# nhchiu/Shadow-Removal-ISTD

Measured on AMD Instinct MI355X. Metric: ST-CGAN train images/s at 256×256 bs=32, 1/2/4/8 MI355X; G2 max-abs vs CPU, higher is better.
Workload: dtype bf16; 1 GPU; full ST-CGAN train step (G1,G2,D1,D2 fwd/bwd + MSE-cGAN/L1 + Adam), 256x256; global_batch=32, per_gpu_batch=32, image_size=256, ngf=64, parallelism=dp1, step_launch=eager

## Files before the change

include/stcgan_hip.h:

```cpp
#ifndef STCGAN_HIP_H
#define STCGAN_HIP_H

#include <stdint.h>

#ifdef __cplusplus
extern "C" {
#endif

enum { STC_F32 = 0, STC_BF16 = 1 };

typedef struct {
  void* p;
  int32_t H, W;
  int64_t bs;
  int64_t rs;
  int32_t ps;
  int32_t co;
  int32_t cs;
  int32_t pad_;
} stc_view;

enum { STC_CONV_S2 = 0, STC_CONV_S1 = 1, STC_CONVT_S2 = 2, STC_CONV_S1_DGRAD = 3 };

int stc_conv_fwd(int dtype, int kind, int B,
// ... 41 lines not shown
                    float* running_var, int64_t* num_batches_tracked, float momentum, float eps, stc_view apply_x,
                    stc_view y1, float slope1, stc_view y2, float slope2, void* workspace, int64_t workspace_bytes,
                    void* stream);

int stc_conv_bwd_act_ok(int dtype, int kind, int B, stc_view dy, int Cin, int Cout, stc_view out, stc_view x,
                        stc_view g_other);
int stc_conv_bwd_act(int dtype, int kind, int B, stc_view dy, int Cin, const void* w_packed, int Cout,
                     stc_view out, stc_view x, float slope_self, stc_view g_other, float slope_other, void* stream);

int stc_conv_fwd_act_ok(int dtype, int kind, int B, stc_view x, int Cin, int Cout, stc_view y1, stc_view y2);
int stc_conv_fwd_act(int dtype, int kind, int B, stc_view x, int Cin, const void* w_packed, int Cout,
                     stc_view y1, float slope1, stc_view y2, float slope2, const float* bias,
                     void* workspace, int64_t workspace_bytes, void* stream);

int stc_set_splitk_inlaunch(int on);

int stc_conv_wgrad(int dtype, int B, int stride,
                   stc_view D, int R,
                   const float* d_scale, const float* d_shift, int d_act, float d_slope,
                   stc_view G, int Cg, int Cg_out,
                   const float* g_scale, const float* g_shift, int g_act, float g_slope,
                   float* dW, void* workspace, int64_t workspace_bytes, void* stream);
int64_t stc_conv_wgrad_workspace(int dtype, int B, int Hd, int Wd, int R, int Cg);
int stc_conv_wgrad_ex(int dtype, int B, int stride,
                      stc_view D, int R,
                      const float* d_scale, const float* d_shift, int d_act, float d_slope,
                      stc_view G, int Cg, int Cg_out,
                      const float* g_scale, const float* g_shift, int g_act, float g_slope,
                      float* dW, const int32_t* force_plan, void* workspace, int64_t workspace_bytes, void* stream);
int stc_conv_wgrad_query(int dtype, int B, int Hd, int Wd, int R, int Cg, const int32_t* force_plan,
// ... 197 lines not shown
```

shadow-removal-istd_amd/csrc/bn.hip:

```cpp
#include <type_traits>

#include "common.hpp"
#include "philox.hpp"

namespace stc {

constexpr int STAT_PIX = 64;

__host__ __device__ inline int stat_chunks(long long P) {
  long long c = (P + STAT_PIX - 1) / STAT_PIX;
  if (c > 1024) c = 1024;
  if (c < 1) c = 1;
  return (int)c;
}

template <typename T> struct VW;
template <> struct VW<float> {
  static constexpr int N = 4;
  __device__ __forceinline__ static void load(const float* p, float* f) {
    const float4 v = *reinterpret_cast<const float4*>(p);
    f[0] = v.x; f[1] = v.y; f[2] = v.z; f[3] = v.w;
  }
  __device__ __forceinline__ static void store(float* p, const float* f) {
    *reinterpret_cast<float4*>(p) = make_float4(f[0], f[1], f[2], f[3]);
// ... 186 lines not shown
    }
    sm = mu;
  }
  const double N = n, mu = sm;
  const double M2 = block_sum256(m2, sh);
  if (threadIdx.x == 0)
    bn_finalize_store(c, N, mu, M2, pre, rmean, rvar, nbt, momentum, eps, mean_o, rstd_o, scale, shift);
}

__device__ __forceinline__ double wave_sum(double v) {
#pragma unroll
  for (int o = 32; o > 0; o >>= 1) v += __shfl_xor(v, o, 64);
  return v;
}

__global__ void __launch_bounds__(256) bn_finalize_wave_kernel(const float* part, int nchunks, int C,
                                                               const float* gamma, const float* beta,
                                                               float* rmean, float* rvar, long long* nbt,
                                                               float momentum, float eps,
                                                               float* mean_o, float* rstd_o, float* scale, float* shift) {
  const int lane = threadIdx.x & 63;
  const int c = blockIdx.x * 4 + (threadIdx.x >> 6);
  if (c >= C) return;
  auto load4 = [&](int k0, float4* pp) {
#pragma unroll
    for (int u = 0; u < 4; ++u) {
      const int k = k0 + u * 64;
      pp[u] = k < nchunks ? *reinterpret_cast<const float4*>(part + ((long long)k * C + c) * 4)
                          : make_float4(0.f, 0.f, 0.f, 0.f);
    }
  };
  const BnPre pre = bn_pre(c, gamma, beta, rmean, rvar);
  auto sum1 = [&](const float4* pp, double& n, double& sm) {
#pragma unroll
    for (int u = 0; u < 4; ++u) {
      if (pp[u].x <= 0.f) continue;
      n += pp[u].x;
      sm += (double)pp[u].x * pp[u].w + (double)pp[u].y;
    }
  };
  auto sum2 = [&](const float4* pp, double mu, double& m2) {
#pragma unroll
    for (int u = 0; u < 4; ++u) {
      if (pp[u].x <= 0.f) continue;
      const double nb = pp[u].x, s1 = pp[u].y, r = s1 / nb;
      double q = (double)pp[u].z - s1 * r;
      if (q < 0) q = 0;
// ... 25 lines not shown
  } else {
    for (int k0 = lane; k0 < nchunks; k0 += 256) {
      float4 pp[4];
      load4(k0, pp);
      sum1(pp, n, sm);
    }
    n = wave_sum(n);
    sm = wave_sum(sm);
    mu = n > 0 ? sm / n : 0.0;
    for (int k0 = lane; k0 < nchunks; k0 += 256) {
      float4 pp[4];
      load4(k0, pp);
      sum2(pp, mu, m2);
    }
  }
  const double M2 = wave_sum(m2);
  if (lane == 0) bn_finalize_store(c, n, mu, M2, pre, rmean, rvar, nbt, momentum, eps, mean_o, rstd_o, scale, shift);
}

__global__ void bn_eval_table_kernel(int C, const float* gamma, const float* beta, const float* rmean,
                                     const float* rvar, float eps, float* scale, float* shift) {
  const int c = blockIdx.x * blockDim.x + threadIdx.x;
  if (c >= C) return;
  const float rs = 1.f / sqrtf(rvar[c] + eps);
  const float sc = gamma[c] * rs;
  scale[c] = sc;
  shift[c] = beta[c] - rmean[c] * sc;
}

struct GradIn {
  View g1, g2;
// ... 95 lines not shown
    }
#pragma unroll
    for (int u = 0; u < 4; ++u) {
      a += pp[u].x;
      b += pp[u].y;
    }
  }
  const double ta = block_sum256(a, sh);
  const double tb = block_sum256(b, sh);
  if (threadIdx.x == 0) {
    dbeta[c] = (float)ta;
    dgamma[c] = (float)tb;
  }
}

__global__ void __launch_bounds__(256) bn_bwd_finalize_wave_kernel(const float* part, int nchunks, int C, float* dgamma,
                                                                   float* dbeta) {
  const int lane = threadIdx.x & 63;
  const int c = blockIdx.x * 4 + (threadIdx.x >> 6);
  if (c >= C) return;
  double a = 0, b = 0;
  for (int k0 = lane; k0 < nchunks; k0 += 256) {
    float2 pp[4];
#pragma unroll
    for (int u = 0; u < 4; ++u) {
      const int k = k0 + u * 64;
      pp[u] = k < nchunks ? *reinterpret_cast<const float2*>(part + ((long long)k * C + c) * 2) : make_float2(0.f, 0.f);
    }
#pragma unroll
    for (int u = 0; u < 4; ++u) {
      a += pp[u].x;
      b += pp[u].y;
    }
  }
  a = wave_sum(a);
  b = wave_sum(b);
  if (lane == 0) {
    dbeta[c] = (float)a;
    dgamma[c] = (float)b;
  }
}

template <typename T, bool DENSE>
__global__ void __launch_bounds__(256) bn_bwd_apply_kernel(View x, PixDiv pd, long long P, int C, const float* scale,
                                                           const float* shift, const float* mean, const float* rstd,
                                                           const float* gamma, GradIn gi, const float* dgamma,
                                                           const float* dbeta, View dx) {
  constexpr int N = VW<T>::N;
  const int CG = C / N;
  const long long total = P * CG;
  const long long stride = (long long)gridDim.x * blockDim.x;
  const float invP = 1.f / (float)P;
  int cg_have = -1;
  float sc[N], sh[N], k0[N], k1[N], k2[N];
  auto table = [&](int cg) {
    if (cg == cg_have) return;
    cg_have = cg;
    const int c = N * cg;
    if (scale) { ldc<N>(scale + c, sc); ldc<N>(shift + c, sh); }
    else {
#pragma unroll
      for (int e = 0; e < N; ++e) { sc[e] = 1.f; sh[e] = 0.f; }
    }
    if (mean) {
      float mu[N], rs[N], gm[N], dg[N], db[N];
      ldc<N>(mean + c, mu); ldc<N>(rstd + c, rs); ldc<N>(gamma + c, gm); ldc<N>(dgamma + c, dg); ldc<N>(dbeta + c, db);
#pragma unroll
      for (int e = 0; e < N; ++e) {
        k1[e] = gm[e] * rs[e];
        k2[e] = k1[e] * rs[e] * dg[e] * invP;
        k0[e] = k1[e] * (db[e] * invP - mu[e] * rs[e] * dg[e] * invP);
      }
    } else {
#pragma unroll
      for (int e = 0; e < N; ++e) { k1[e] = 1.f; k2[e] = 0.f; k0[e] = 0.f; }
    }
  };
  struct Off {
    long long x, g1, g2, dx;
    int c;
  };
  auto offs = [&](long long idx) {
    Off o;
    const int cg = (int)(idx % CG);
    const long long pix = idx / CG;
    o.c = N * cg;
    if constexpr (DENSE) {
// ... 10 lines not shown
      o.dx = vidx(dx, b, yy, xx, o.c);
    }
    return o;
  };
  struct In {
    float v[N], g1[N], g2[N];
  };
  auto load = [&](const Off& o, In& in) {
    VW<T>::load(reinterpret_cast<const T*>(x.p) + o.x, in.v);
    if (gi.has1) VW<T>::load(reinterpret_cast<const T*>(gi.g1.p) + o.g1, in.g1);
    if (gi.has2) VW<T>::load(reinterpret_cast<const T*>(gi.g2.p) + o.g2, in.g2);
  };
  auto emit = [&](const Off& o, const In& in) {
    table(o.c / N);
    float d[N];
#pragma unroll
    for (int e = 0; e < N; ++e) {
      const float n = fmaf(in.v[e], sc[e], sh[e]);
      float dn = 0.f;
      if (gi.has1) dn += in.g1[e] * dact(n, gi.s1);
      if (gi.has2) dn += in.g2[e] * dact(n, gi.s2);
      d[e] = fmaf(k1[e], dn, -fmaf(k2[e], in.v[e], k0[e]));
    }
    VW<T>::store(reinterpret_cast<T*>(dx.p) + o.dx, d);
  };
  if constexpr (DENSE) {
    const unsigned nthr = gridDim.x * blockDim.x, t0 = blockIdx.x * blockDim.x + threadIdx.x;
    const unsigned pstep = nthr / (unsigned)CG, Pu = (unsigned)P;
    unsigned pix = t0 / (unsigned)CG;
    if (pix >= Pu) return;
    const int c = N * (int)(t0 % (unsigned)CG);
    table(c / N);
    const T* xp = reinterpret_cast<const T*>(x.p) + x.co + c;
    const T* g1p = reinterpret_cast<const T*>(gi.g1.p) + gi.g1.co + c;
    const T* g2p = reinterpret_cast<const T*>(gi.g2.p) + gi.g2.co + c;
    T* dp = reinterpret_cast<T*>(dx.p) + dx.co + c;
    const unsigned xs = x.ps, g1s = gi.g1.ps, g2s = gi.g2.ps, ds = dx.ps;
    auto ld = [&](unsigned q, In& in) {
      VW<T>::load(xp + q * xs, in.v);
      if (gi.has1) VW<T>::load(g1p + q * g1s, in.g1);
      if (gi.has2) VW<T>::load(g2p + q * g2s, in.g2);
    };
    auto put = [&](unsigned q, const In& in) {
      float d[N];
#pragma unroll
      for (int e = 0; e < N; ++e) {
        const float n = fmaf(in.v[e], sc[e], sh[e]);
        float dn = 0.f;
        if (gi.has1) dn += in.g1[e] * dact(n, gi.s1);
        if (gi.has2) dn += in.g2[e] * dact(n, gi.s2);
        d[e] = fmaf(k1[e], dn, -fmaf(k2[e], in.v[e], k0[e]));
      }
      VW<T>::store(dp + q * ds, d);
    };
    for (; pix + pstep < Pu; pix += 2 * pstep) {
      In a, b;
      ld(pix, a);
      ld(pix + pstep, b);
      put(pix, a);
      put(pix + pstep, b);
    }
    if (pix < Pu) {
      In a;
      ld(pix, a);
      put(pix, a);
    }
    return;
  }
  long long idx = (long long)blockIdx.x * blockDim.x + threadIdx.x;
  for (; idx + stride < total; idx += 2 * stride) {
    const Off oa = offs(idx), ob = offs(idx + stride);
    In a, b;
    load(oa, a);
    load(ob, b);
    emit(oa, a);
    emit(ob, b);
  }
  if (idx < total) {
    const Off oa = offs(idx);
    In a;
    load(oa, a);
    emit(oa, a);
  }
}

template <typename T, bool DENSE>
__global__ void __launch_bounds__(256) bn_apply_kernel(View x, PixDiv pd, long long P, int C, const float* scale,
                                                       const float* shift, View y1, float s1, View y2, float s2,
                                                       int has2) {
  constexpr int N = VW<T>::N;
  const int CG = C / N;
  const long long total = P * CG;
  const long long stride = (long long)gridDim.x * blockDim.x;
  int cg_have = -1;
  float sc[N], sh[N];
  auto table = [&](int cg) {
    if (cg == cg_have) return;
// ... 9 lines not shown
    const long long pix = idx / CG;
    c = N * cg;
    if constexpr (DENSE) {
      ox = pix * x.ps + x.co + c;
      o1 = pix * y1.ps + y1.co + c;
      o2 = pix * y2.ps + y2.co + c;
    } else {
      int b, yy, xx;
      pix_bxy(pd, pix, b, yy, xx);
      ox = vidx(x, b, yy, xx, c);
      o1 = vidx(y1, b, yy, xx, c);
      o2 = vidx(y2, b, yy, xx, c);
    }
  };
  auto emit = [&](const float* v0, long long o1, long long o2) {
    float v[N], o[N];
#pragma unroll
    for (int e = 0; e < N; ++e) v[e] = fmaf(v0[e], sc[e], sh[e]);
#pragma unroll
    for (int e = 0; e < N; ++e) o[e] = act(v[e], s1);
    VW<T>::store(reinterpret_cast<T*>(y1.p) + o1, o);
    if (has2) {
#pragma unroll
      for (int e = 0; e < N; ++e) o[e] = act(v[e], s2);
      VW<T>::store(reinterpret_cast<T*>(y2.p) + o2, o);
    }
  };
  if constexpr (DENSE) {
    const unsigned nthr = gridDim.x * blockDim.x, t0 = blockIdx.x * blockDim.x + threadIdx.x;
    const unsigned pstep = nthr / (unsigned)CG, Pu = (unsigned)P;
    unsigned pix = t0 / (unsigned)CG;
    if (pix >= Pu) return;
    const int c = N * (int)(t0 % (unsigned)CG);
    table(c / N);
    const T* xp = reinterpret_cast<const T*>(x.p) + x.co + c;
    const unsigned xs = x.ps, s1s = y1.ps, s2s = y2.ps;
    const long long b1 = y1.co + c, b2 = y2.co + c;
    for (; pix + pstep < Pu; pix += 2 * pstep) {
      float va[N], vb[N];
      VW<T>::load(xp + pix * xs, va);
      VW<T>::load(xp + (pix + pstep) * xs, vb);
// ... 17 lines not shown
    VW<T>::load(reinterpret_cast<const T*>(x.p) + ax, va);
    VW<T>::load(reinterpret_cast<const T*>(x.p) + bx, vb);
    table(ca / N);
    emit(va, a1, a2);
    table(cb / N);
    emit(vb, b1, b2);
  }
  if (idx < total) {
    long long ax, a1, a2;
    int ca;
    offs(idx, ax, a1, a2, ca);
    float va[N];
    VW<T>::load(reinterpret_cast<const T*>(x.p) + ax, va);
    table(ca / N);
    emit(va, a1, a2);
  }
}

template <typename T>
__global__ void __launch_bounds__(256) chan_sum_kernel(View x, PixDiv pd, long long P, int C, float* part, int nchunks) {
  constexpr int N = VW<T>::N;
  const int CG = C / N;
  const int RL = 256 / CG;
  const int cg = threadIdx.x % CG, pl = threadIdx.x / CG;
  const long long per = (P + nchunks - 1) / nchunks;
  const long long p0 = blockIdx.x * per, p1 = min(P, p0 + per);
  __shared__ float red[256][N];
  float a[N];
#pragma unroll
  for (int e = 0; e < N; ++e) a[e] = 0.f;
// ... 365 lines not shown
    STC_CHECK_LAUNCH();
  }
  View v = mkview(x), o = mkview(dx);
  const PixDiv pd = mkpix(B, x.H, x.W);
  const long long P = (long long)B * x.H * x.W;
  const int N = dtype == STC_F32 ? 4 : 8;
  const long long work = P * (C / N);
  const bool dense = stream_ok(B, x, C, N) && stream_ok(B, dx, C, N) && stream_ok(B, g1, C, N) && stream_ok(B, g2, C, N);
  const int blocks = dense ? grid_stream(work) : grid_for(work);
#define STC_BB(T_, D_) hipLaunchKernelGGL((bn_bwd_apply_kernel<T_, D_>), dim3(blocks), dim3(256), 0, st, v, pd, P, C, scale, shift, mean, rstd, gamma, gi, dgamma, dbeta, o)
  if (dtype == STC_F32) { if (dense) STC_BB(float, true); else STC_BB(float, false); }
  else { if (dense) STC_BB(bf16, true); else STC_BB(bf16, false); }
#undef STC_BB
  STC_CHECK_LAUNCH();
  return 0;
}

static int mkdrop(const stc_dropout* d, int B, int C, DropDev* out, const char* who) {
  STC_REQUIRE(d && d->state, "%s: dropout block with a device {seed, offset} required", who);
  STC_REQUIRE(d->p >= 0.0 && d->p < 1.0, "%s: drop probability %g outside [0, 1)", who, d->p);
  STC_REQUIRE(d->level >= 0 && d->H > 0 && d->W > 0 && B > 0 && C > 0 && C % 4 == 0,
              "%s: bad dropout level %d / extent %d x %d x %d x %d (C %% 4 == 0)", who, d->level, B, d->H, d->W, C);
  STC_REQUIRE((long long)B * d->H * d->W * C < (1ll << 34), "%s: more than 2^34 elements under one dropout level", who);
  out->state = reinterpret_cast<const unsigned long long*>(d->state);
  out->level = (unsigned)d->level;
  out->thresh = (unsigned)(unsigned long long)(d->p * 4294967296.0);
  out->scale = (float)(1.0 / (1.0 - d->p));
  out->H = d->H; out->W = d->W;
  return 0;
}
// ... 120 lines not shown
```

shadow-removal-istd_amd/csrc/common.hpp:

```cpp
#pragma once
#include <hip/hip_runtime.h>
#include <hip/hip_bf16.h>
#include <stdint.h>
#include <string>
#include <cstdio>
#include <cstdarg>

#include "../../include/stcgan_hip.h"

namespace stc {

using bf16 = __hip_bfloat16;
typedef float floatx4 __attribute__((ext_vector_type(4)));
typedef float floatx16 __attribute__((ext_vector_type(16)));
typedef short shortx8 __attribute__((ext_vector_type(8)));
typedef short shortx4 __attribute__((ext_vector_type(4)));

#ifndef STC_EXP_NODMA
#define STC_EXP_NODMA 0
#endif
#ifndef STC_EXP_NOMFMA
#define STC_EXP_NOMFMA 0
#endif
#ifndef STC_EXP_NOEPI
// ... 84 lines not shown
};
static inline View mkview(const stc_view& v) {
  View r;
  r.p = (char*)v.p; r.H = v.H; r.W = v.W; r.bs = v.bs; r.rs = v.rs;
  r.ps = v.ps; r.co = v.co; r.cs = v.cs;
  return r;
}
__device__ __forceinline__ long long vidx(const View& v, int b, int y, int x, int c) {
  return (long long)b * v.bs + (long long)y * v.rs + (long long)x * v.ps + (long long)(v.co + c) * v.cs;
}

__device__ __forceinline__ float act(float v, float slope) { return v > 0.f ? v : v * slope; }
__device__ __forceinline__ float dact(float n, float slope) { return n > 0.f ? 1.f : slope; }

static inline int cdiv(long long a, long long b) { return (int)((a + b - 1) / b); }

__device__ __forceinline__ int fast_div(int n, int d, float inv) {
  int q = (int)((float)n * inv);
  const int r = n - q * d;
  return q + (r >= d) - (r < 0);
}

struct Geometry {
  int taps_lg_tw;
  int in_stride, os, nphase;
  int offy[4], offx[4];
  int stepy, stepx;
};

static inline Geometry geometry(int kind) {
// ... 13 lines not shown
      for (int z = 0; z < 4; ++z) { g.offy[z] = z >> 1; g.offx[z] = z & 1; }
      g.stepy = -1; g.stepx = -1;
      break;
  }
  return g;
}

struct BnPre {
  float g, bt, rm, rv;
};
__device__ __forceinline__ BnPre bn_pre(int c, const float* gamma, const float* beta, const float* rmean,
                                        const float* rvar) {
  return BnPre{gamma ? gamma[c] : 1.f, beta ? beta[c] : 0.f, rmean ? rmean[c] : 0.f, rvar ? rvar[c] : 0.f};
}

__device__ __forceinline__ void bn_finalize_store(int c, double N, double mu, double M2, const BnPre& q, float* rmean,
                                                  float* rvar, long long* nbt, float momentum, float eps,
                                                  float* mean_o, float* rstd_o, float* scale, float* shift) {
  const double var = N > 0 ? M2 / N : 0.0;
  const float rs = (float)(1.0 / sqrt(var + (double)eps));
  if (mean_o) mean_o[c] = (float)mu;
  if (rstd_o) rstd_o[c] = rs;
  const float sc = q.g * rs;
  scale[c] = sc;
  shift[c] = q.bt - (float)mu * sc;
  if (rmean) rmean[c] = (1.f - momentum) * q.rm + momentum * (float)mu;
  if (rvar) rvar[c] = (1.f - momentum) * q.rv + momentum * (float)(N > 1 ? M2 / (N - 1) : var);
  if (nbt && c == 0) nbt[0] += 1;
}
__device__ __forceinline__ void bn_finalize_store(int c, double N, double mu, double M2, const float* gamma,
                                                  const float* beta, float* rmean, float* rvar, long long* nbt,
                                                  float momentum, float eps, float* mean_o, float* rstd_o,
                                                  float* scale, float* shift) {
  bn_finalize_store(c, N, mu, M2, bn_pre(c, gamma, beta, rmean, rvar), rmean, rvar, nbt, momentum, eps, mean_o,
                    rstd_o, scale, shift);
}

}
```

shadow-removal-istd_amd/csrc/igemm.hip:

```cpp
#include "common.hpp"

namespace stc {

struct ConvParams {
  const char* a;
  long long a_bs, a_rs;
  int a_ps, a_co;
  int IH, IW;
  int cin, lg_tw, in_stride;
  int offy[4], offx[4];
  int stepy, stepx;
  const float* sc;
  const float* sh;
  int pro_act;
  float slope;
  int GH, GW, M, N, K;
  int ksplit, kchunk;
  const char* b;
  long long b_phase_stride;
  char* c;
  long long c_bs, c_rs;
  int c_ps, c_co, c_cs;
  int os;
  int oy0[4], ox0[4];
// ... 684 lines not shown
  if (rc != 0 || stats_part == nullptr) return rc;
  STC_REQUIRE(!out_f32 || dtype == STC_F32, "stc_conv_fwd_ex: stats of a non-activation output");
  return stc_chan_stats(dtype, B, y, Cout, stats_part, stats_chunks, stream);
}

extern "C" int stc_conv_bn_fwd(int dtype, int kind, int B, stc_view x, int Cin, const void* w_packed, int Cout,
                               stc_view y, float* fws, int nchunks, const float* gamma, const float* beta,
                               float* running_mean, float* running_var, int64_t* num_batches_tracked, float momentum,
                               float eps, stc_view apply_x, stc_view y1, float slope1, stc_view y2, float slope2,
                               void* workspace, int64_t workspace_bytes, void* stream) {
  STC_REQUIRE(fws && nchunks > 0 && gamma && beta, "stc_conv_bn_fwd: statistics workspace and BN affine required");
  int rc = stc_conv_fwd_ex(dtype, kind, B, x, Cin, w_packed, Cout, y, nullptr, 0, 0, fws, nchunks, nullptr, workspace,
                           workspace_bytes, stream);
  if (rc) return rc;
  float* tab = fws + (int64_t)nchunks * Cout * 4;
  rc = stc_bn_finalize(fws, nchunks, Cout, gamma, beta, running_mean, running_var, num_batches_tracked, momentum, eps,
                       tab, tab + Cout, tab + 2 * Cout, tab + 3 * Cout, stream);
  if (rc || !y1.p) return rc;
  return stc_bn_apply(dtype, B, apply_x, Cout, tab + 2 * Cout, tab + 3 * Cout, y1, slope1, y2, slope2, stream);
}

extern "C" int stc_conv_fwd(int dtype, int kind, int B, stc_view x, int Cin,
                            const float* pro_scale, const float* pro_shift, int pro_act, float pro_slope,
                            const void* w_packed, int Cout, stc_view y,
                            const float* bias, int epi_tanh, int out_f32,
                            void* workspace, int64_t workspace_bytes, void* stream) {
  STC_REQUIRE(dtype == STC_F32 || dtype == STC_BF16, "stc_conv_fwd: bad dtype %d", dtype);
  STC_REQUIRE(kind >= 0 && kind <= 3, "stc_conv_fwd: bad kind %d", kind);
  const int VEC = dtype == STC_F32 ? 4 : 8;
  const int BK = dtype == STC_F32 ? 32 : 64;
// ... 119 lines not shown
  return stc_bn_bwd_reduce(dtype, B, bnb->x, bnb->C, bnb->scale, bnb->shift, bnb->mean, bnb->rstd, g1, bnb->slope_self,
                           bnb->g_other, bnb->slope_other, part2, need, stream);
}

extern "C" int stc_conv_bwd_bn_apply(int dtype, int kind, int B, stc_view dy, int Cin, const void* w_packed, int Cout,
                                     stc_view out, const stc_bnb_fuse* bnb, float* part2, int nchunks,
                                     const float* gamma, stc_view dx, float* dgamma, float* dbeta, void* workspace,
                                     int64_t workspace_bytes, void* stream) {
  int rc = stc_conv_bwd_bn(dtype, kind, B, dy, Cin, w_packed, Cout, out, bnb, part2, nchunks, workspace,
                           workspace_bytes, stream);
  if (rc) return rc;
  stc_view g1 = out;
  g1.co += bnb->ch_off;
  g1.H = bnb->x.H;
  g1.W = bnb->x.W;
  return stc_bn_bwd_apply(dtype, B, bnb->x, bnb->C, bnb->scale, bnb->shift, bnb->mean, bnb->rstd, gamma, g1,
                          bnb->slope_self, bnb->g_other, bnb->slope_other, part2, nchunks, dx, dgamma, dbeta, stream);
}

namespace stc {
bool bf16_conv_bwd_act_ok(int kind, int B, const stc_view& dy, int Cin, int Cout, const stc_view& out, const stc_view& x,
                          const stc_view* g_other);
}
extern "C" int stc_conv_bwd_act_ok(int dtype, int kind, int B, stc_view dy, int Cin, int Cout, stc_view out, stc_view x,
                                   stc_view g_other) {
  if (kind < 0 || kind > 3 || !bf16_path(dtype, kind, Cin, Cout)) return 0;
  return bf16_conv_bwd_act_ok(kind, B, dy, Cin, Cout, out, x, &g_other) ? 1 : 0;
}

extern "C" int stc_conv_bwd_act(int dtype, int kind, int B, stc_view dy, int Cin, const void* w_packed, int Cout,
// ... 29 lines not shown
```

shadow-removal-istd_amd/stcgan_amd/_lib.py:

```python
import ctypes
import os

import torch

_HERE = os.path.dirname(os.path.abspath(__file__))
LIB_PATH = os.environ.get("STC_LIB_PATH") or os.path.join(_HERE, "libstcgan_hip.so")

F32, BF16 = 0, 1
CONV_S2, CONV_S1, CONVT_S2, CONV_S1_DGRAD = 0, 1, 2, 3
PACK_CONV_FWD, PACK_CONV_DGRAD, PACK_CONV_S1_DGRAD, PACK_CONVT_FWD, PACK_CONVT_DGRAD = 0, 1, 2, 3, 4
LOSS_L1, LOSS_MSE_CONST, LOSS_BCE_CONST = 0, 1, 2
LOSS_COMBINE_D, LOSS_COMBINE_G = 0, 1


class View(ctypes.Structure):
    _fields_ = [("p", ctypes.c_void_p), ("H", ctypes.c_int32), ("W", ctypes.c_int32),
                ("bs", ctypes.c_int64), ("rs", ctypes.c_int64), ("ps", ctypes.c_int32),
                ("co", ctypes.c_int32), ("cs", ctypes.c_int32), ("pad_", ctypes.c_int32)]


NULL_VIEW = View(None, 0, 0, 0, 0, 0, 0, 1, 0)

PACK_MAX = 40

# ... 36 lines not shown
    "stc_conv_fwd_query": (_i32, [_i32, _i32, _i32, _i32, _i32, _i32, _i32, _i32, _vp, _vp, _vp, _vp]),
    "stc_conv_bwd_bn_chunks": (_i32, [_i32, _i32, _i32, _i32, _i32, _i32, _i32, _i32, _i32]),
    "stc_conv_bwd_bn_chunks_ex": (_i32, [_i32, _i32, _i32, View, _i32, _i32, View, _vp]),
    "stc_conv_bwd_bn": (_i32, [_i32, _i32, _i32, View, _i32, _vp, _i32, View, _vp, _vp, _i32, _vp, _i64, _vp]),
    "stc_conv_fwd_ex": (_i32, [_i32, _i32, _i32, View, _i32, _vp, _i32, View, _vp, _i32, _i32, _vp, _i32, _vp, _vp,
                               _i64, _vp]),
    "stc_conv_fwd_act_ok": (_i32, [_i32, _i32, _i32, View, _i32, _i32, View, View]),
    "stc_conv_fwd_act": (_i32, [_i32, _i32, _i32, View, _i32, _vp, _i32, View, _f32, View, _f32, _vp, _vp, _i64, _vp]),
    "stc_conv_bwd_bn_apply": (_i32, [_i32, _i32, _i32, View, _i32, _vp, _i32, View, _vp, _vp, _i32, _vp, View, _vp,
                                     _vp, _vp, _i64, _vp]),
    "stc_conv_bn_fwd": (_i32, [_i32, _i32, _i32, View, _i32, _vp, _i32, View, _vp, _i32, _vp, _vp, _vp, _vp, _vp, _f32,
                               _f32, View, View, _f32, View, _f32, _vp, _i64, _vp]),
    "stc_conv_bwd_act_ok": (_i32, [_i32, _i32, _i32, View, _i32, _i32, View, View, View]),
    "stc_conv_bwd_act": (_i32, [_i32, _i32, _i32, View, _i32, _vp, _i32, View, View, _f32, View, _f32, _vp]),
    "stc_set_splitk_inlaunch": (_i32, [_i32]),
    "stc_conv_wgrad": (_i32, [_i32, _i32, _i32, View, _i32, _vp, _vp, _i32, _f32, View, _i32, _i32, _vp, _vp, _i32,
                              _f32, _vp, _vp, _i64, _vp]),
    "stc_conv_wgrad_workspace": (_i64, [_i32, _i32, _i32, _i32, _i32, _i32]),
    "stc_conv_wgrad_ex": (_i32, [_i32, _i32, _i32, View, _i32, _vp, _vp, _i32, _f32, View, _i32, _i32, _vp, _vp, _i32,
                                 _f32, _vp, _vp, _vp, _i64, _vp]),
    "stc_conv_wgrad_query": (_i32, [_i32, _i32, _i32, _i32, _i32, _i32, _vp, _vp, _vp]),
    "stc_pack_weight": (_i32, [_i32, _i32, _vp, _i32, _i32, _vp, _i32, _i32, _vp]),
    "stc_pack_weights": (_i32, [_i32, _i32, _vp, _vp]),
    "stc_chan_stats": (_i32, [_i32, _i32, View, _i32, _vp, _i32, _vp]),
    "stc_chan_stats_chunks": (_i32, [_i32, _i32, _i32]),
    "stc_chan_sum": (_i32, [_i32, _i32, View, _i32, _i32, _vp, _i32, _vp, _vp]),
    "stc_bn_apply": (_i32, [_i32, _i32, View, _i32, _vp, _vp, View, _f32, View, _f32, _vp]),
    "stc_bn_finalize": (_i32, [_vp, _i32, _i32, _vp, _vp, _vp, _vp, _vp, _f32, _f32, _vp, _vp, _vp, _vp, _vp]),
    "stc_bn_bwd_reduce": (_i32, [_i32, _i32, View, _i32, _vp, _vp, _vp, _vp, View, _f32, View, _f32, _vp, _i32,
                                 _vp]),
# ... 137 lines not shown
```

shadow-removal-istd_amd/stcgan_amd/ops.py:

```python
import ctypes

import torch

from . import _lib as L
from ._lib import check, lib, ptr, stream

LRELU = 0.2
BN_EPS = 1e-5
BN_MOMENTUM = 0.1


def vec(dt):
    return 4 if dt == torch.float32 else 8


def pad_channels(c, dt):
    p = vec(dt)
    while p < c:
        p *= 2
    return p


def _ws(nbytes, device):
    if nbytes <= 0:
# ... 29 lines not shown
_MEMO = {}


def _conv_ws_bytes(kind, B, gh, gw, cin, cout, dt):
    key = ("cws", kind, B, gh, gw, cin, cout, dt)
    v = _MEMO.get(key)
    if v is None:
        v = _MEMO[key] = lib().stc_conv_fwd_workspace(L.dtype_code(dt), kind, B, gh, gw, cin, cout)
    return v


def set_splitk_inlaunch(on):
    old = bool(lib().stc_set_splitk_inlaunch(1 if on else 0))
    _MEMO.clear()
    return old


def plan_of(kind, B, gh, gw, cin, cout, dt):
    out = (ctypes.c_int32 * 4)()
    check(lib().stc_conv_fwd_plan(L.dtype_code(dt), kind, B, gh, gw, cin, cout, out), "stc_conv_fwd_plan")
    return tuple(out)


def conv(kind, B, xv, cin, w_packed, cout, yv, dt, pro=None, slope=None, bias=None, tanh=False, out_f32=False,
         force=None):
    dev = w_packed.device
    if kind == L.CONVT_S2:
        gh, gw = xv.H, xv.W
    else:
        gh, gw = yv.H, yv.W
# ... 798 lines not shown
```

Before: 3121 images/s.

## Fuse BN finalize with apply for small-spatial tail layers

Adds fused kernels for BatchNorm layers with few pixels (P ≤ 2048), such as the deep encoder/decoder layers. In the forward pass the per-chunk statistics merge, the scale/shift table computation and the normalize+activation apply run in one launch. In the backward pass the dgamma/dbeta reduction and the dx apply are fused the same way. This removes a kernel launch and a global round trip per small BN layer, at the cost of every pixel-slice block redundantly re-merging the partial statistics for its channel group. The path is on by default and can be toggled or queried from Python.

```diff
diff --git a/include/stcgan_hip.h b/include/stcgan_hip.h
--- a/include/stcgan_hip.h
+++ b/include/stcgan_hip.h
@@ -79,6 +79,9 @@
                      void* workspace, int64_t workspace_bytes, void* stream);
 
 int stc_set_splitk_inlaunch(int on);
+
+int stc_set_bn_tail(int on);
+int stc_bn_tail_query(int dtype, int B, int H, int W, int C, int nchunks, int backward);
 
 int stc_conv_wgrad(int dtype, int B, int stride,
                    stc_view D, int R,
diff --git a/shadow-removal-istd_amd/csrc/bn.hip b/shadow-removal-istd_amd/csrc/bn.hip
--- a/shadow-removal-istd_amd/csrc/bn.hip
+++ b/shadow-removal-istd_amd/csrc/bn.hip
@@ -224,14 +224,8 @@
   return v;
 }
 
-__global__ void __launch_bounds__(256) bn_finalize_wave_kernel(const float* part, int nchunks, int C,
-                                                               const float* gamma, const float* beta,
-                                                               float* rmean, float* rvar, long long* nbt,
-                                                               float momentum, float eps,
-                                                               float* mean_o, float* rstd_o, float* scale, float* shift) {
-  const int lane = threadIdx.x & 63;
-  const int c = blockIdx.x * 4 + (threadIdx.x >> 6);
-  if (c >= C) return;
+__device__ __forceinline__ void bn_merge_wave(const float* part, int nchunks, int C, int c, int lane, double& n_o,
+                                              double& mu_o, double& M2_o) {
   auto load4 = [&](int k0, float4* pp) {
 #pragma unroll
     for (int u = 0; u < 4; ++u) {
@@ -240,7 +234,6 @@
                           : make_float4(0.f, 0.f, 0.f, 0.f);
     }
   };
-  const BnPre pre = bn_pre(c, gamma, beta, rmean, rvar);
   auto sum1 = [&](const float4* pp, double& n, double& sm) {
 #pragma unroll
     for (int u = 0; u < 4; ++u) {
@@ -296,7 +289,22 @@
       sum2(pp, mu, m2);
     }
   }
-  const double M2 = wave_sum(m2);
+  n_o = n;
+  mu_o = mu;
+  M2_o = wave_sum(m2);
+}
+
+__global__ void __launch_bounds__(256) bn_finalize_wave_kernel(const float* part, int nchunks, int C,
+                                                               const float* gamma, const float* beta,
+                                                               float* rmean, float* rvar, long long* nbt,
+                                                               float momentum, float eps,
+                                                               float* mean_o, float* rstd_o, float* scale, float* shift) {
+  const int lane = threadIdx.x & 63;
+  const int c = blockIdx.x * 4 + (threadIdx.x >> 6);
+  if (c >= C) return;
+  const BnPre pre = bn_pre(c, gamma, beta, rmean, rvar);
+  double n, mu, M2;
+  bn_merge_wave(part, nchunks, C, c, lane, n, mu, M2);
   if (lane == 0) bn_finalize_store(c, n, mu, M2, pre, rmean, rvar, nbt, momentum, eps, mean_o, rstd_o, scale, shift);
 }
 
@@ -422,30 +430,60 @@
   }
 }
 
+__device__ __forceinline__ void bn_bwd_merge_wave(const float* part, int nchunks, int C, int c, int lane, double& a_o,
+                                                  double& b_o) {
+  double a = 0, b = 0;
+  for (int k0 = lane; k0 < nchunks; k0 += 256) {
+    float2 pp[4];
+#pragma unroll
+    for (int u = 0; u < 4; ++u) {
+      const int k = k0 + u * 64;
+      pp[u] = k < nchunks ? *reinterpret_cast<const float2*>(part + ((long long)k * C + c) * 2) : make_float2(0.f, 0.f);
+    }
+#pragma unroll
+    for (int u = 0; u < 4; ++u) {
+      a += pp[u].x;
+      b += pp[u].y;
+    }
+  }
+  a_o = wave_sum(a);
+  b_o = wave_sum(b);
+}
+
 __global__ void __launch_bounds__(256) bn_bwd_finalize_wave_kernel(const float* part, int nchunks, int C, float* dgamma,
                                                                    float* dbeta) {
   const int lane = threadIdx.x & 63;
   const int c = blockIdx.x * 4 + (threadIdx.x >> 6);
   if (c >= C) return;
-  double a = 0, b = 0;
-  for (int k0 = lane; k0 < nchunks; k0 += 256) {
-    float2 pp[4];
-#pragma unroll
-    for (int u = 0; u < 4; ++u) {
-      const int k = k0 + u * 64;
-      pp[u] = k < nchunks ? *reinterpret_cast<const float2*>(part + ((long long)k * C + c) * 2) : make_float2(0.f, 0.f);
-    }
-#pragma unroll
-    for (int u = 0; u < 4; ++u) {
-      a += pp[u].x;
-      b += pp[u].y;
-    }
-  }
-  a = wave_sum(a);
-  b = wave_sum(b);
+  double a, b;
+  bn_bwd_merge_wave(part, nchunks, C, c, lane, a, b);
   if (lane == 0) {
     dbeta[c] = (float)a;
     dgamma[c] = (float)b;
+  }
+}
+
+template <int N>
+__device__ __forceinline__ void bn_bwd_coef(const float* mu, const float* rs, const float* gm, const float* dg,
+                                            const float* db, float invP, float* k0, float* k1, float* k2) {
+#pragma unroll
+  for (int e = 0; e < N; ++e) {
+    k1[e] = gm[e] * rs[e];
+    k2[e] = k1[e] * rs[e] * dg[e] * invP;
+    k0[e] = k1[e] * (db[e] * invP - mu[e] * rs[e] * dg[e] * invP);
+  }
+}
+template <int N>
+__device__ __forceinline__ void bn_bwd_elem(const float* v, const float* g1, const float* g2, int has1, int has2,
+                                            float s1, float s2, const float* sc, const float* sh, const float* k0,
+                                            const float* k1, const float* k2, float* d) {
+#pragma unroll
+  for (int e = 0; e < N; ++e) {
+    const float n = fmaf(v[e], sc[e], sh[e]);
+    float dn = 0.f;
+    if (has1) dn += g1[e] * dact(n, s1);
+    if (has2) dn += g2[e] * dact(n, s2);
+    d[e] = fmaf(k1[e], dn, -fmaf(k2[e], v[e], k0[e]));
   }
 }
 
@@ -473,12 +511,7 @@
     if (mean) {
       float mu[N], rs[N], gm[N], dg[N], db[N];
       ldc<N>(mean + c, mu); ldc<N>(rstd + c, rs); ldc<N>(gamma + c, gm); ldc<N>(dgamma + c, dg); ldc<N>(dbeta + c, db);
-#pragma unroll
-      for (int e = 0; e < N; ++e) {
-        k1[e] = gm[e] * rs[e];
-        k2[e] = k1[e] * rs[e] * dg[e] * invP;
-        k0[e] = k1[e] * (db[e] * invP - mu[e] * rs[e] * dg[e] * invP);
-      }
+      bn_bwd_coef<N>(mu, rs, gm, dg, db, invP, k0, k1, k2);
     } else {
 #pragma unroll
       for (int e = 0; e < N; ++e) { k1[e] = 1.f; k2[e] = 0.f; k0[e] = 0.f; }
@@ -519,14 +552,7 @@
   auto emit = [&](const Off& o, const In& in) {
     table(o.c / N);
     float d[N];
-#pragma unroll
-    for (int e = 0; e < N; ++e) {
-      const float n = fmaf(in.v[e], sc[e], sh[e]);
-      float dn = 0.f;
-      if (gi.has1) dn += in.g1[e] * dact(n, gi.s1);
-      if (gi.has2) dn += in.g2[e] * dact(n, gi.s2);
-      d[e] = fmaf(k1[e], dn, -fmaf(k2[e], in.v[e], k0[e]));
-    }
+    bn_bwd_elem<N>(in.v, in.g1, in.g2, gi.has1, gi.has2, gi.s1, gi.s2, sc, sh, k0, k1, k2, d);
     VW<T>::store(reinterpret_cast<T*>(dx.p) + o.dx, d);
   };
   if constexpr (DENSE) {
@@ -548,14 +574,7 @@
     };
     auto put = [&](unsigned q, const In& in) {
       float d[N];
-#pragma unroll
-      for (int e = 0; e < N; ++e) {
-        const float n = fmaf(in.v[e], sc[e], sh[e]);
-        float dn = 0.f;
-        if (gi.has1) dn += in.g1[e] * dact(n, gi.s1);
-        if (gi.has2) dn += in.g2[e] * dact(n, gi.s2);
-        d[e] = fmaf(k1[e], dn, -fmaf(k2[e], in.v[e], k0[e]));
-      }
+      bn_bwd_elem<N>(in.v, in.g1, in.g2, gi.has1, gi.has2, gi.s1, gi.s2, sc, sh, k0, k1, k2, d);
       VW<T>::store(dp + q * ds, d);
     };
     for (; pix + pstep < Pu; pix += 2 * pstep) {
@@ -586,6 +605,23 @@
     In a;
     load(oa, a);
     emit(oa, a);
+  }
+}
+
+template <typename T>
+__device__ __forceinline__ void bn_act_emit(const float* v0, const float* sc, const float* sh, float s1, float s2,
+                                            int has2, T* p1, T* p2) {
+  constexpr int N = VW<T>::N;
+  float v[N], o[N];
+#pragma unroll
+  for (int e = 0; e < N; ++e) v[e] = fmaf(v0[e], sc[e], sh[e]);
+#pragma unroll
+  for (int e = 0; e < N; ++e) o[e] = act(v[e], s1);
+  VW<T>::store(p1, o);
+  if (has2) {
+#pragma unroll
+    for (int e = 0; e < N; ++e) o[e] = act(v[e], s2);
+    VW<T>::store(p2, o);
   }
 }
 
@@ -625,17 +661,7 @@
     }
   };
   auto emit = [&](const float* v0, long long o1, long long o2) {
-    float v[N], o[N];
-#pragma unroll
-    for (int e = 0; e < N; ++e) v[e] = fmaf(v0[e], sc[e], sh[e]);
-#pragma unroll
-    for (int e = 0; e < N; ++e) o[e] = act(v[e], s1);
-    VW<T>::store(reinterpret_cast<T*>(y1.p) + o1, o);
-    if (has2) {
-#pragma unroll
-      for (int e = 0; e < N; ++e) o[e] = act(v[e], s2);
-      VW<T>::store(reinterpret_cast<T*>(y2.p) + o2, o);
-    }
+    bn_act_emit<T>(v0, sc, sh, s1, s2, has2, reinterpret_cast<T*>(y1.p) + o1, reinterpret_cast<T*>(y2.p) + o2);
   };
   if constexpr (DENSE) {
     const unsigned nthr = gridDim.x * blockDim.x, t0 = blockIdx.x * blockDim.x + threadIdx.x;
@@ -683,6 +709,118 @@
     VW<T>::load(reinterpret_cast<const T*>(x.p) + ax, va);
     table(ca / N);
     emit(va, a1, a2);
+  }
+}
+
+constexpr int TAIL_THREADS = 512;
+constexpr int TAIL_PIX = 2;
+constexpr int TAIL_SLICE = TAIL_THREADS * TAIL_PIX;
+
+__device__ __forceinline__ int tail_group(int id, int G) { return (G & 7) ? id : (id & 7) * (G >> 3) + (id >> 3); }
+
+template <typename T>
+__global__ void __launch_bounds__(TAIL_THREADS) bn_tail_fwd_kernel(const float* part, int nchunks, int C,
+                                                                   const float* gamma, const float* beta, float* rmean,
+                                                                   float* rvar, long long* nbt, float momentum,
+                                                                   float eps, float* mean_o, float* rstd_o, float* scale,
+                                                                   float* shift, View x, PixDiv pd, int P, View y1,
+                                                                   float s1, View y2, float s2, int has2) {
+  constexpr int N = VW<T>::N;
+  __shared__ float tab[N][2];
+  const int lane = threadIdx.x & 63;
+  const int c0 = tail_group(blockIdx.x, gridDim.x) * N;
+  const bool first = blockIdx.y == 0;
+  for (int j = threadIdx.x >> 6; j < N; j += TAIL_THREADS / 64) {
+    const int c = c0 + j;
+    const BnPre pre = bn_pre(c, gamma, beta, first ? rmean : nullptr, first ? rvar : nullptr);
+    double n, mu, M2;
+    bn_merge_wave(part, nchunks, C, c, lane, n, mu, M2);
+    if (lane == 0) {
+      const BnTab t = bn_table_of(n, mu, M2, pre, eps);
+      tab[j][0] = t.sc;
+      tab[j][1] = t.sf;
+      if (first)
+        bn_finalize_store(c, n, mu, M2, pre, rmean, rvar, nbt, momentum, eps, mean_o, rstd_o, scale, shift);
+    }
+  }
+  __syncthreads();
+  float sc[N], sh[N];
+#pragma unroll
+  for (int e = 0; e < N; ++e) { sc[e] = tab[e][0]; sh[e] = tab[e][1]; }
+  const int pend = min(P, ((int)blockIdx.y + 1) * TAIL_SLICE);
+  const int p0 = blockIdx.y * TAIL_SLICE + threadIdx.x;
+  float v[TAIL_PIX][N];
+  long long o1[TAIL_PIX], o2[TAIL_PIX];
+#pragma unroll
+  for (int u = 0; u < TAIL_PIX; ++u) {
+    const int pix = p0 + u * TAIL_THREADS;
+    if (pix >= pend) break;
+    int b, yy, xx;
+    pix_bxy(pd, pix, b, yy, xx);
+    VW<T>::load(vptr<T>(x, b, yy, xx, c0), v[u]);
+    o1[u] = vidx(y1, b, yy, xx, c0);
+    o2[u] = vidx(y2, b, yy, xx, c0);
+  }
+#pragma unroll
+  for (int u = 0; u < TAIL_PIX; ++u) {
+    if (p0 + u * TAIL_THREADS >= pend) break;
+    bn_act_emit<T>(v[u], sc, sh, s1, s2, has2, reinterpret_cast<T*>(y1.p) + o1[u], reinterpret_cast<T*>(y2.p) + o2[u]);
+  }
+}
+
+template <typename T>
+__global__ void __launch_bounds__(TAIL_THREADS) bn_tail_bwd_kernel(const float* part, int nchunks, int C, float* dgamma,
+                                                                   float* dbeta, View x, PixDiv pd, int P,
+                                                                   const float* scale, const float* shift,
+                                                                   const float* mean, const float* rstd,
+                                                                   const float* gamma, GradIn gi, View dx) {
+  constexpr int N = VW<T>::N;
+  __shared__ float tab[2][N];
+  const int lane = threadIdx.x & 63;
+  const int c0 = tail_group(blockIdx.x, gridDim.x) * N;
+  for (int j = threadIdx.x >> 6; j < N; j += TAIL_THREADS / 64) {
+    const int c = c0 + j;
+    double a, b;
+    bn_bwd_merge_wave(part, nchunks, C, c, lane, a, b);
+    if (lane == 0) {
+      const float db = (float)a, dg = (float)b;
+      tab[0][j] = dg;
+      tab[1][j] = db;
+      if (blockIdx.y == 0) {
+        dbeta[c] = db;
+        dgamma[c] = dg;
+      }
+    }
+  }
+  float sc[N], sh[N], mu[N], rs[N], gm[N];
+  ldc<N>(scale + c0, sc); ldc<N>(shift + c0, sh); ldc<N>(mean + c0, mu); ldc<N>(rstd + c0, rs); ldc<N>(gamma + c0, gm);
+  __syncthreads();
+  float dg[N], db[N], k0[N], k1[N], k2[N];
+#pragma unroll
+  for (int e = 0; e < N; ++e) { dg[e] = tab[0][e]; db[e] = tab[1][e]; }
+  const float invP = 1.f / (float)P;
+  bn_bwd_coef<N>(mu, rs, gm, dg, db, invP, k0, k1, k2);
+  const int pend = min(P, ((int)blockIdx.y + 1) * TAIL_SLICE);
+  const int p0 = blockIdx.y * TAIL_SLICE + threadIdx.x;
+  float v[TAIL_PIX][N], g1[TAIL_PIX][N], g2[TAIL_PIX][N];
+  long long od[TAIL_PIX];
+#pragma unroll
+  for (int u = 0; u < TAIL_PIX; ++u) {
+    const int pix = p0 + u * TAIL_THREADS;
+    if (pix >= pend) break;
+    int b, yy, xx;
+    pix_bxy(pd, pix, b, yy, xx);
+    VW<T>::load(vptr<T>(x, b, yy, xx, c0), v[u]);
+    if (gi.has1) VW<T>::load(vptr<T>(gi.g1, b, yy, xx, c0), g1[u]);
+    if (gi.has2) VW<T>::load(vptr<T>(gi.g2, b, yy, xx, c0), g2[u]);
+    od[u] = vidx(dx, b, yy, xx, c0);
+  }
+#pragma unroll
+  for (int u = 0; u < TAIL_PIX; ++u) {
+    if (p0 + u * TAIL_THREADS >= pend) break;
+    float d[N];
+    bn_bwd_elem<N>(v[u], g1[u], g2[u], gi.has1, gi.has2, gi.s1, gi.s2, sc, sh, k0, k1, k2, d);
+    VW<T>::store(reinterpret_cast<T*>(dx.p) + od[u], d);
   }
 }
 
@@ -1078,6 +1216,67 @@
 #undef STC_BB
   STC_CHECK_LAUNCH();
   return 0;
+}
+
+constexpr int kBnTailPixels = 2048;
+static int g_bn_tail = kBnTailPixels;
+extern "C" int stc_set_bn_tail(int on) {
+  const int old = g_bn_tail == kBnTailPixels ? 1 : g_bn_tail;
+  if (on >= 0) g_bn_tail = on == 1 ? kBnTailPixels : std::min(on, 1 << 20);
+  return old;
+}
+
+namespace stc {
+bool bn_tail_ok(int dtype, long long P, int C, int nchunks, bool backward) {
+  const int N = dtype == STC_F32 ? 4 : 8;
+  return g_bn_tail > 0 && (dtype == STC_F32 || dtype == STC_BF16) && P > 0 && P <= g_bn_tail && C > 0 && C % N == 0 &&
+         nchunks > 0 && nchunks <= (backward ? 256 : 1024);
+}
+
+int bn_tail_fwd(int dtype, int B, const float* part, int nchunks, int C, const float* gamma, const float* beta,
+                float* running_mean, float* running_var, int64_t* num_batches_tracked, float momentum, float eps,
+                float* mean, float* rstd, float* scale, float* shift, stc_view x, stc_view y1, float slope1,
+                stc_view y2, float slope2, hipStream_t st) {
+  const long long P = (long long)B * x.H * x.W;
+  STC_REQUIRE(part && scale && shift && y1.p && bn_tail_ok(dtype, P, C, nchunks, false), "bn_tail_fwd: not a tail layer");
+  STC_REQUIRE(vec_ok(dtype, C, x) && vec_ok(dtype, C, y1) && (!y2.p || vec_ok(dtype, C, y2)),
+              "bn_tail_fwd: C=%d / views not 16-byte vectorisable NHWC", C);
+  const int N = dtype == STC_F32 ? 4 : 8;
+  View v = mkview(x), o1 = mkview(y1), o2 = y2.p ? mkview(y2) : mkview(y1);
+  const PixDiv pd = mkpix(B, x.H, x.W);
+  const int h2 = y2.p != nullptr ? 1 : 0;
+  const int slices = (int)((P + TAIL_SLICE - 1) / TAIL_SLICE);
+#define STC_TF(T_) hipLaunchKernelGGL(bn_tail_fwd_kernel<T_>, dim3(C / N, slices), dim3(TAIL_THREADS), 0, st, part, nchunks, C, gamma, beta, running_mean, running_var, (long long*)num_batches_tracked, momentum, eps, mean, rstd, scale, shift, v, pd, (int)P, o1, slope1, o2, slope2, h2)
+  if (dtype == STC_F32) STC_TF(float); else STC_TF(bf16);
+#undef STC_TF
+  STC_CHECK_LAUNCH();
+  return 0;
+}
+
+int bn_tail_bwd(int dtype, int B, stc_view x, int C, const float* scale, const float* shift, const float* mean,
+                const float* rstd, const float* gamma, stc_view g1, float slope1, stc_view g2, float slope2,
+                const float* part2, int nchunks, stc_view dx, float* dgamma, float* dbeta, hipStream_t st) {
+  const long long P = (long long)B * x.H * x.W;
+  STC_REQUIRE(bn_tail_ok(dtype, P, C, nchunks, true), "bn_tail_bwd: not a tail layer");
+  STC_REQUIRE(vec_ok(dtype, C, x) && vec_ok(dtype, C, dx) && (!g1.p || vec_ok(dtype, C, g1)) &&
+                  (!g2.p || vec_ok(dtype, C, g2)),
+              "bn_tail_bwd: bad C=%d / views", C);
+  STC_REQUIRE(mean && part2 && dgamma && dbeta && gamma && rstd && scale && shift, "bn_tail_bwd: missing BN tensors");
+  const int N = dtype == STC_F32 ? 4 : 8;
+  GradIn gi = mkgrad(g1, slope1, g2, slope2);
+  View v = mkview(x), o = mkview(dx);
+  const PixDiv pd = mkpix(B, x.H, x.W);
+  const int slices = (int)((P + TAIL_SLICE - 1) / TAIL_SLICE);
+#define STC_TB(T_) hipLaunchKernelGGL(bn_tail_bwd_kernel<T_>, dim3(C / N, slices), dim3(TAIL_THREADS), 0, st, part2, nchunks, C, dgamma, dbeta, v, pd, (int)P, scale, shift, mean, rstd, gamma, gi, o)
+  if (dtype == STC_F32) STC_TB(float); else STC_TB(bf16);
+#undef STC_TB
+  STC_CHECK_LAUNCH();
+  return 0;
+}
+}
+
+extern "C" int stc_bn_tail_query(int dtype, int B, int H, int W, int C, int nchunks, int backward) {
+  return bn_tail_ok(dtype, (long long)B * H * W, C, nchunks, backward != 0) ? 1 : 0;
 }
 
 static int mkdrop(const stc_dropout* d, int B, int C, DropDev* out, const char* who) {
diff --git a/shadow-removal-istd_amd/csrc/common.hpp b/shadow-removal-istd_amd/csrc/common.hpp
--- a/shadow-removal-istd_amd/csrc/common.hpp
+++ b/shadow-removal-istd_amd/csrc/common.hpp
@@ -122,6 +122,15 @@
 __device__ __forceinline__ float dact(float n, float slope) { return n > 0.f ? 1.f : slope; }
 
 static inline int cdiv(long long a, long long b) { return (int)((a + b - 1) / b); }
+
+bool bn_tail_ok(int dtype, long long P, int C, int nchunks, bool backward);
+int bn_tail_fwd(int dtype, int B, const float* part, int nchunks, int C, const float* gamma, const float* beta,
+                float* running_mean, float* running_var, int64_t* num_batches_tracked, float momentum, float eps,
+                float* mean, float* rstd, float* scale, float* shift, stc_view x, stc_view y1, float slope1,
+                stc_view y2, float slope2, hipStream_t st);
+int bn_tail_bwd(int dtype, int B, stc_view x, int C, const float* scale, const float* shift, const float* mean,
+                const float* rstd, const float* gamma, stc_view g1, float slope1, stc_view g2, float slope2,
+                const float* part2, int nchunks, stc_view dx, float* dgamma, float* dbeta, hipStream_t st);
 
 __device__ __forceinline__ int fast_div(int n, int d, float inv) {
   int q = (int)((float)n * inv);
@@ -165,16 +174,25 @@
   return BnPre{gamma ? gamma[c] : 1.f, beta ? beta[c] : 0.f, rmean ? rmean[c] : 0.f, rvar ? rvar[c] : 0.f};
 }
 
+struct BnTab {
+  float rs, sc, sf;
+};
+__device__ __forceinline__ BnTab bn_table_of(double N, double mu, double M2, const BnPre& q, float eps) {
+  const double var = N > 0 ? M2 / N : 0.0;
+  const float rs = (float)(1.0 / sqrt(var + (double)eps));
+  const float sc = q.g * rs;
+  return BnTab{rs, sc, q.bt - (float)mu * sc};
+}
+
 __device__ __forceinline__ void bn_finalize_store(int c, double N, double mu, double M2, const BnPre& q, float* rmean,
                                                   float* rvar, long long* nbt, float momentum, float eps,
                                                   float* mean_o, float* rstd_o, float* scale, float* shift) {
   const double var = N > 0 ? M2 / N : 0.0;
-  const float rs = (float)(1.0 / sqrt(var + (double)eps));
+  const BnTab t = bn_table_of(N, mu, M2, q, eps);
   if (mean_o) mean_o[c] = (float)mu;
-  if (rstd_o) rstd_o[c] = rs;
-  const float sc = q.g * rs;
-  scale[c] = sc;
-  shift[c] = q.bt - (float)mu * sc;
+  if (rstd_o) rstd_o[c] = t.rs;
+  scale[c] = t.sc;
+  shift[c] = t.sf;
   if (rmean) rmean[c] = (1.f - momentum) * q.rm + momentum * (float)mu;
   if (rvar) rvar[c] = (1.f - momentum) * q.rv + momentum * (float)(N > 1 ? M2 / (N - 1) : var);
   if (nbt && c == 0) nbt[0] += 1;
diff --git a/shadow-removal-istd_amd/csrc/igemm.hip b/shadow-removal-istd_amd/csrc/igemm.hip
--- a/shadow-removal-istd_amd/csrc/igemm.hip
+++ b/shadow-removal-istd_amd/csrc/igemm.hip
@@ -722,6 +722,10 @@
                            workspace_bytes, stream);
   if (rc) return rc;
   float* tab = fws + (int64_t)nchunks * Cout * 4;
+  if (y1.p && bn_tail_ok(dtype, (long long)B * apply_x.H * apply_x.W, Cout, nchunks, false))
+    return bn_tail_fwd(dtype, B, fws, nchunks, Cout, gamma, beta, running_mean, running_var, num_batches_tracked,
+                       momentum, eps, tab, tab + Cout, tab + 2 * Cout, tab + 3 * Cout, apply_x, y1, slope1, y2, slope2,
+                       (hipStream_t)stream);
   rc = stc_bn_finalize(fws, nchunks, Cout, gamma, beta, running_mean, running_var, num_batches_tracked, momentum, eps,
                        tab, tab + Cout, tab + 2 * Cout, tab + 3 * Cout, stream);
   if (rc || !y1.p) return rc;
@@ -871,6 +875,10 @@
   g1.co += bnb->ch_off;
   g1.H = bnb->x.H;
   g1.W = bnb->x.W;
+  if (bnb->mean && bn_tail_ok(dtype, (long long)B * bnb->x.H * bnb->x.W, bnb->C, nchunks, true))
+    return bn_tail_bwd(dtype, B, bnb->x, bnb->C, bnb->scale, bnb->shift, bnb->mean, bnb->rstd, gamma, g1,
+                       bnb->slope_self, bnb->g_other, bnb->slope_other, part2, nchunks, dx, dgamma, dbeta,
+                       (hipStream_t)stream);
   return stc_bn_bwd_apply(dtype, B, bnb->x, bnb->C, bnb->scale, bnb->shift, bnb->mean, bnb->rstd, gamma, g1,
                           bnb->slope_self, bnb->g_other, bnb->slope_other, part2, nchunks, dx, dgamma, dbeta, stream);
 }
diff --git a/shadow-removal-istd_amd/stcgan_amd/_lib.py b/shadow-removal-istd_amd/stcgan_amd/_lib.py
--- a/shadow-removal-istd_amd/stcgan_amd/_lib.py
+++ b/shadow-removal-istd_amd/stcgan_amd/_lib.py
@@ -74,6 +74,8 @@
     "stc_conv_bwd_act_ok": (_i32, [_i32, _i32, _i32, View, _i32, _i32, View, View, View]),
     "stc_conv_bwd_act": (_i32, [_i32, _i32, _i32, View, _i32, _vp, _i32, View, View, _f32, View, _f32, _vp]),
     "stc_set_splitk_inlaunch": (_i32, [_i32]),
+    "stc_set_bn_tail": (_i32, [_i32]),
+    "stc_bn_tail_query": (_i32, [_i32, _i32, _i32, _i32, _i32, _i32, _i32]),
     "stc_conv_wgrad": (_i32, [_i32, _i32, _i32, View, _i32, _vp, _vp, _i32, _f32, View, _i32, _i32, _vp, _vp, _i32,
                               _f32, _vp, _vp, _i64, _vp]),
     "stc_conv_wgrad_workspace": (_i64, [_i32, _i32, _i32, _i32, _i32, _i32]),
diff --git a/shadow-removal-istd_amd/stcgan_amd/ops.py b/shadow-removal-istd_amd/stcgan_amd/ops.py
--- a/shadow-removal-istd_amd/stcgan_amd/ops.py
+++ b/shadow-removal-istd_amd/stcgan_amd/ops.py
@@ -67,6 +67,14 @@
     old = bool(lib().stc_set_splitk_inlaunch(1 if on else 0))
     _MEMO.clear()
     return old
+
+
+def set_bn_tail(on):
+    return lib().stc_set_bn_tail(int(on))
+
+
+def bn_tail_takes(B, H, W, C, nch, dt, backward=False):
+    return bool(lib().stc_bn_tail_query(L.dtype_code(dt), B, H, W, C, nch, int(backward)))
 
 
 def plan_of(kind, B, gh, gw, cin, cout, dt):
```

New measurement: 3087 images/s. 1.1% lower.
